# CliMA/OrthogonalSphericalShellGrids.jl

Hardware: AMD Instinct MI355X
Metric: grid-cells/s metric precompute + zipper halo-fill GB/s, 1/10°×75z (higher is better)
Workload: dtype f64

## Files before the change

orthogonalsphericalshellgrids.jl_amd/csrc/tpg_api.hip:

```cpp
#include "tpg_common.hpp"
#include <string.h>
#include <stdlib.h>
#include <atomic>
#include <mutex>

namespace tpg {

static thread_local char g_err[512] = "";

void set_error(const char* fmt, ...)
{
    va_list ap;
    va_start(ap, fmt);
    vsnprintf(g_err, sizeof(g_err), fmt, ap);
    va_end(ap);
}

#ifdef TPG_TEST_ABI
static std::atomic<const Config*> g_config{nullptr};
static std::mutex g_config_mutex;

static int env_int(const char* name, int dflt)
{
    const char* e = getenv(name);
    return (e && *e) ? atoi(e) : dflt;
}

static const Config* read_config()
{
    Config* c = new Config;
    c->cells_variant = env_int("TPG_CELLS_VARIANT", 2) == 0 ? 0 : 2;
    c->build_nt = env_int("TPG_BUILD_NT", 1) != 0;
    c->zipper_variant = env_int("TPG_ZIPPER_VARIANT", 3) == 0 ? 0 : 3;
    c->fill_fused = env_int("TPG_FILL_FUSED", -1);
    c->fill_merged = env_int("TPG_FILL_MERGED", -1);
    c->exchange_in_capture = env_int("TPG_EXCHANGE_IN_CAPTURE", 0) != 0;
    c->exchange_fail_stage = env_int("TPG_EXCHANGE_FAIL_STAGE", -1);
    const char* lib = getenv("TPG_RCCL_LIBRARY");
    c->rccl_library = (lib && *lib) ? strdup(lib) : nullptr;
    return c;
}

const Config& config()
{
    const Config* c = g_config.load(std::memory_order_acquire);
    if (!c) {
        std::lock_guard<std::mutex> lock(g_config_mutex);
        c = g_config.load(std::memory_order_acquire);
        if (!c) { c = read_config(); g_config.store(c, std::memory_order_release); }
    }
    return *c;
}
#else
const Config& config()
{
    static const Config k{ 2, true, 3, -1, -1, false, -1, nullptr };
    return k;
}
#endif

int check_geom(int Nx, int Ny, int Nz, int Hx, int Hy, int Hz, int ft)
{
    if (ft != TPG_F32 && ft != TPG_F64) { set_error("unknown element type ft=%d", ft); return TPG_ERR_INVALID_ARGUMENT; }
    if (Nx < 2 || Ny < 1 || Nz < 1 || Hx < 0 || Hy < 0 || Hz < 0) {
        set_error("invalid size (%d,%d,%d) / halo (%d,%d,%d)", Nx, Ny, Nz, Hx, Hy, Hz);
        return TPG_ERR_INVALID_ARGUMENT;
    }
    if (Nx % 2) {
        set_error("The number of cells in the longitude dimension should be even!");
        return TPG_ERR_ODD_NLAMBDA;
    }
    if (Hx > Nx || Hy > Ny) {
        set_error("halo (%d,%d) larger than size (%d,%d)", Hx, Hy, Nx, Ny);
        return TPG_ERR_UNSUPPORTED;
    }
    if ((long long)(Nx + 2 * Hx) * (Ny + 2 * Hy) >= (1ll << 31) || (long long)Nx * (Nz + 2 * Hz) * (Hy + 1) >= (1ll << 31)) {
        set_error("horizontal plane too large for 32-bit indexing");
        return TPG_ERR_UNSUPPORTED;
    }
    return TPG_OK;
}

}

extern "C" {

int tpg_version(void) { return TPG_VERSION; }

#ifdef TPG_TEST_ABI
int tpg_reload_config(void)
{
    std::lock_guard<std::mutex> lock(tpg::g_config_mutex);
    tpg::g_config.store(tpg::read_config(), std::memory_order_release);
    return TPG_OK;
}
#endif

const char* tpg_last_error(void) { return tpg::g_err; }

const char* tpg_status_string(int status)
{
    switch (status) {
    case TPG_OK: return "ok";
    case TPG_ERR_INVALID_ARGUMENT: return "invalid argument";
    case TPG_ERR_ODD_NLAMBDA: return "The number of cells in the longitude dimension should be even!";
    case TPG_ERR_BAD_PARTITION: return "latitude band outside the global grid (only y-partitioning is supported)";
    case TPG_ERR_WORKSPACE: return "workspace missing or too small";
    case TPG_ERR_UNSUPPORTED: return "unsupported size";
    case TPG_ERR_NOT_NORTH: return "Zipper boundary condition is valid on the north side only";
    case TPG_ERR_RCCL: return "RCCL error (librccl missing or ncclResult_t failure)";
    default: return status > 0 ? hipGetErrorString((hipError_t)status) : "unknown status";
    }
}

}
```

orthogonalsphericalshellgrids.jl_amd/csrc/tpg_grid.hip:

```cpp
#include "tpg_common.hpp"
#include "tpg_math.hpp"
#include "tpg_batch.hpp"

using namespace tpgm;

namespace {

constexpr double kC180Pi = 180.0 / kPi;
constexpr double kC360Pi = 360.0 / kPi;

struct GridK {
    int Nx, Ny, Hx, Hy;
    int shift;
    int jstart, jend;
    int jm_lo, jm_hi;
    int sx, rows;
    int ft;
    double fplp90;
    double R;
    const double* ti;
    const double* tj;
    const double* ts;
};

struct OutPtrs { void* p[TPG_NUM_ARRAYS]; };

struct TableArgs {
    int Nx, Ny, Hy, shift, ft;
    double south, npl, R;
    double* ti; double* tj; double* ts;
};

__device__ double lambda_face(int i, int N, int ft)
{
    long long num = 360ll * (i - 1) - 180ll * N;
    if (ft == TPG_F32) return (double)((float)num / (float)N);
    return (double)num / (double)N;
}
__device__ double lambda_center(int i, int N, int ft)
{
    long long num = 360ll * (2ll * i - 1) - 360ll * N;
    if (ft == TPG_F32) return (double)((float)num / (float)(2ll * N));
    return (double)num / (double)(2ll * N);
}
__device__ double phi_center(int j, int N, double south)
{
    if (N == 1) return south;
    if (south == __builtin_rint(south) && absD(south) < 1e6) {
        long long s = (long long)south;
        long long num = s * (N - 1) + (90 - s) * (long long)(j - 1);
        return (double)num / (double)(N - 1);
    }
    dd step = dd_div(two_sum(90.0, -south), dd{ (double)(N - 1), 0.0 });
    dd v = dd_add(dd{ south, 0.0 }, dd_mul_d(step, (double)(j - 1)));
    return v.hi + v.lo;
}

__global__ __launch_bounds__(64) void k_tables(TableArgs t)
{
    int tid = blockIdx.x * blockDim.x + threadIdx.x;
    const double a = tand((90.0 - t.npl) / 2);
    if (tid < t.Nx) {
        int is = tid + 1;
        int i0 = is - t.shift; if (i0 < 1) i0 += t.Nx;
        double lf = lambda_face(i0, t.Nx, t.ft), lc = lambda_center(i0, t.Nx, t.ft);
        double slf = sind(lf), clf = cosd(lf), slc = sind(lc), clc = cosd(lc);
        if (t.ft == TPG_F32) {
            slf = (double)(float)slf; clf = (double)(float)clf; slc = (double)(float)slc; clc = (double)(float)clc;
        }
        t.ti[0 * t.Nx + tid] = a * slf;
        t.ti[1 * t.Nx + tid] = a * clf;
        t.ti[2 * t.Nx + tid] = a * slc;
        t.ti[3 * t.Nx + tid] = a * clc;
        return;
    }
    tid -= t.Nx;
    if (tid < 2 * t.Ny) {
        int face = tid < t.Ny;
        int j = (face ? tid : tid - t.Ny) + 1;
        double pc = phi_center(j, t.Ny, t.south);
        double phi = pc;
        if (face) {
            double dphi = t.Ny > 1 ? phi_center(2, t.Ny, t.south) - phi_center(1, t.Ny, t.south) : 0.0;
            phi = pc - dphi / 2;
        }
        double psi = asinhD(tand((90.0 - phi) / 2) / a);
        double sh, ch;
        sinh_cosh(psi, sh, ch);
        int base = face ? 0 : 2;
        t.tj[(base + 0) * t.Ny + (j - 1)] = sh;
        t.tj[(base + 1) * t.Ny + (j - 1)] = ch;
        return;
    }
    tid -= 2 * t.Ny;
    if (tid <= t.Hy) {
        int j = 1 - t.Hy + tid;
        const double south = t.south, R = t.R;
        const double dlam = 360.0 / (double)t.Nx;
        const double dphiL = (90.0 - south) / (double)t.Ny;
        double pf, pfn, pc, pcm;
        if (south == __builtin_rint(south)) {
            long long s = (long long)south, Ny = t.Ny;
            pf  = (double)(s * Ny + (90 - s) * (long long)(j - 1)) / (double)Ny;
            pfn = (double)(s * Ny + (90 - s) * (long long)j) / (double)Ny;
            pc  = (double)(2 * s * Ny + (90 - s) * (long long)(2 * j - 1)) / (double)(2 * Ny);
            pcm = (double)(2 * s * Ny + (90 - s) * (long long)(2 * j - 3)) / (double)(2 * Ny);
        } else {
            pf  = south + (double)(j - 1) * dphiL;
            pfn = south + (double)j * dphiL;
            pc  = south + ((double)(2 * j - 1) * (90.0 - south)) / (double)(2 * t.Ny);
            pcm = south + ((double)(2 * j - 3) * (90.0 - south)) / (double)(2 * t.Ny);
        }
        int n = t.Hy + 1;
        t.ts[0 * n + tid] = R * (dlam * kDeg2Rad) * cosD(kPi * pc / 180);
        t.ts[1 * n + tid] = R * (dlam * kDeg2Rad) * cosD(kPi * pf / 180);
        t.ts[2 * n + tid] = R * R * (dlam * kDeg2Rad) * (sinD(kPi * pfn / 180) - sinD(kPi * pf / 180));
        t.ts[3 * n + tid] = R * R * (dlam * kDeg2Rad) * (sinD(kPi * pc / 180) - sinD(kPi * pcm / 180));
        t.ts[4 * n + tid] = R * (dphiL * kDeg2Rad);
    }
}

struct LP { double lam, phi; };

__device__ __forceinline__ LP analytic(const GridK& g, int xl, int yl, int is, int js)
{
    int i0 = is - g.shift; if (i0 < 1) i0 += g.Nx;
    const double* ti = g.ti + (xl == TPG_FACE ? 0 : 2) * g.Nx;
    const double* tj = g.tj + (yl == TPG_FACE ? 0 : 2) * g.Ny;
    double asl = ti[is - 1], acl = ti[g.Nx + is - 1];
    double sh = tj[js - 1], ch = tj[g.Ny + js - 1];
    double x = asl * ch;
    double y = acl * sh;
    bool pole = (x == 0.0) & (y == 0.0);
    double l = pole ? (i0 == 1 ? -90.0 : 90.0) : -kC180Pi * atanD(y / x);
    LP r;
    r.phi = 90.0 - kC360Pi * atanD(sqrt(y * y + x * x));
    l += (i0 <= g.Nx / 2) ? -90.0 : 90.0;
    l += g.fplp90;
    r.lam = fmod360(fmod360(l) + 360.0);
    return r;
}

__device__ __forceinline__ int fold_partner(int xl, int i, int Nx)
{
    int ip = (xl == TPG_FACE) ? Nx - i + 2 : Nx - i + 1;
    return ip > Nx ? ip - Nx : ip;
}

__device__ __forceinline__ LP coord(const GridK& g, int xl, int yl, int i, int j)
{
    if (j < 1) return LP{ 0.0, 0.0 };
    int iw = i < 1 ? i + g.Nx : (i > g.Nx ? i - g.Nx : i);
    int js = j;
    if (j > g.Ny) {
        int dj = j - g.Ny;
        js = (yl == TPG_FACE) ? g.Ny - dj + 1 : g.Ny - dj;
        iw = fold_partner(xl, iw, g.Nx);
        if (js < 1) return LP{ 0.0, 0.0 };
    } else if (j == g.Ny && yl == TPG_CENTER && iw > g.Nx / 2) {
        iw = fold_partner(xl, iw, g.Nx);
    }
    return analytic(g, xl, yl, iw, js);
}

__device__ __forceinline__ double haversine(LP a, LP b, double R)
{
    double dl = (b.lam - a.lam) * kDeg2Rad;
    double a1 = a.phi * kDeg2Rad;
    double a2 = b.phi * kDeg2Rad;
    double dp = a2 - a1;
    double s1 = sinD(dp / 2), s2 = sinD(dl / 2);
    double h = s1 * s1 + cosD(a1) * cosD(a2) * (s2 * s2);
    double r = sqrt(h);
    return 2 * (R * asinD(r != r ? r : (r < 1.0 ? r : 1.0)));
}

struct V3 { double x, y, z; };
__device__ __forceinline__ V3 cartesian(LP p)
{
    double cl = cosd(p.phi);
    return V3{ cosd(p.lam) * cl, sind(p.lam) * cl, sind(p.phi) };
}
__device__ __forceinline__ double dot3(V3 a, V3 b) { return a.x * b.x + a.y * b.y + a.z * b.z; }
__device__ __forceinline__ V3 cross3(V3 a, V3 b)
{
    return V3{ a.y * b.z - a.z * b.y, a.z * b.x - a.x * b.z, a.x * b.y - a.y * b.x };
}
__device__ __forceinline__ double tri_area(V3 a, V3 b, V3 c)
{
    double t = absD(dot3(a, cross3(b, c)));
    t /= 1 + dot3(a, b) + dot3(b, c) + dot3(a, c);
    return 2 * atanD(t);
}
__device__ __forceinline__ double quad_area(V3 a, V3 b, V3 c, V3 d)
{
    double A = tri_area(a, b, c);
    A += tri_area(a, b, d);
    A += tri_area(a, c, d);
    A += tri_area(b, c, d);
    return A / 2;
}

__device__ __forceinline__ double tri_tan_nr(V3 a, V3 b, V3 c)
{
    return div_nr(absD(dot3(a, cross3(b, c))), 1 + dot3(a, b) + dot3(b, c) + dot3(a, c));
}
__device__ __forceinline__ double tri_tan(V3 a, V3 b, V3 c)
{
    return absD(dot3(a, cross3(b, c))) / (1 + dot3(a, b) + dot3(b, c) + dot3(a, c));
}

template <typename T, bool NT = false>
__device__ __forceinline__ void put(const OutPtrs& o, int q, long long off, double v)
{
    T* p = static_cast<T*>(o.p[q]) + off;
    if (NT) __builtin_nontemporal_store((T)v, p); else *p = (T)v;
}

template <typename T, bool NT = false>
__device__ __forceinline__ void put32(const OutPtrs& o, int q, unsigned boff, double v)
{
    asm volatile("" : "+v"(boff));
    T* p = reinterpret_cast<T*>(static_cast<char*>(o.p[q]) + boff);
    if (NT) __builtin_nontemporal_store((T)v, p); else *p = (T)v;
}

template <typename T, bool NT>
__global__ __launch_bounds__(256) void k_cells(GridK g, OutPtrs o)
{
    const int nbx = (g.Nx + 255) / 256;
    int rb = blockIdx.x / nbx;
    int i = (blockIdx.x - rb * nbx) * 256 + threadIdx.x + 1;
    int j = g.jm_lo + rb;
    if (i > g.Nx) return;

    LP cc = coord(g, 0, 0, i, j), fc = coord(g, 1, 0, i, j), cf = coord(g, 0, 1, i, j), ff = coord(g, 1, 1, i, j);
    LP fc_e = coord(g, 1, 0, i + 1, j), fc_s = coord(g, 1, 0, i, j - 1);
    LP cc_w = coord(g, 0, 0, i - 1, j), cc_s = coord(g, 0, 0, i, j - 1), cc_sw = coord(g, 0, 0, i - 1, j - 1);
    LP ff_e = coord(g, 1, 1, i + 1, j), ff_n = coord(g, 1, 1, i, j + 1), ff_ne = coord(g, 1, 1, i + 1, j + 1);
    LP cf_w = coord(g, 0, 1, i - 1, j), cf_n = coord(g, 0, 1, i, j + 1);

    const double R = g.R;
    double dxcc = haversine(fc_e, fc, R);
    double dxfc = haversine(cc, cc_w, R);
    double dxcf = haversine(ff_e, ff, R);
    double dxff = haversine(cf, cf_w, R);
    double dycc = haversine(cf_n, cf, R);
    double dyfc = haversine(ff_n, ff, R);
    double dycf = haversine(cc, cc_s, R);
    double dyff = haversine(fc, fc_s, R);
    double azcc = quad_area(cartesian(ff), cartesian(ff_e), cartesian(ff_ne), cartesian(ff_n)) * (R * R);
    double azfc = dyfc * dxfc;
    double azcf = dycf * dxcf;
    double azff = quad_area(cartesian(cc_sw), cartesian(cc_s), cartesian(cc), cartesian(cc_w)) * (R * R);

    long long off = (long long)(i + g.Hx - 1) + (long long)g.sx * (j - g.jstart + g.Hy);
    put<T, NT>(o, TPG_LAMBDA_CC, off, cc.lam); put<T, NT>(o, TPG_LAMBDA_FC, off, fc.lam);
    put<T, NT>(o, TPG_LAMBDA_CF, off, cf.lam); put<T, NT>(o, TPG_LAMBDA_FF, off, ff.lam);
    put<T, NT>(o, TPG_PHI_CC, off, cc.phi); put<T, NT>(o, TPG_PHI_FC, off, fc.phi);
    put<T, NT>(o, TPG_PHI_CF, off, cf.phi); put<T, NT>(o, TPG_PHI_FF, off, ff.phi);
    put<T, NT>(o, TPG_DX_CC, off, dxcc); put<T, NT>(o, TPG_DX_FC, off, dxfc);
    put<T, NT>(o, TPG_DX_CF, off, dxcf); put<T, NT>(o, TPG_DX_FF, off, dxff);
    put<T, NT>(o, TPG_DY_CC, off, dycc); put<T, NT>(o, TPG_DY_CF, off, dycf);
    put<T, NT>(o, TPG_DY_FC, off, dyfc); put<T, NT>(o, TPG_DY_FF, off, dyff);
    put<T, NT>(o, TPG_AZ_CC, off, azcc); put<T, NT>(o, TPG_AZ_FC, off, azfc);
    put<T, NT>(o, TPG_AZ_CF, off, azcf); put<T, NT>(o, TPG_AZ_FF, off, azff);
}

struct Pt  { double lam, phi, a, ca; };
struct PtX { double lam, phi, a, ca, X, Y, Z; };
struct Nb  { double lam, a, ca; };
struct NbX { double lam, a, ca, X, Y, Z; };

__device__ __forceinline__ Pt make_pt(const GridK& g, int xl, int yl, int i, int j)
{
    LP p = coord(g, xl, yl, i, j);
    Pt r; r.lam = p.lam; r.phi = p.phi; r.a = p.phi * kDeg2Rad; r.ca = cosD(r.a);
    return r;
}
__device__ __forceinline__ PtX make_ptx(const GridK& g, int xl, int yl, int i, int j)
{
    LP p = coord(g, xl, yl, i, j);
    PtX r; r.lam = p.lam; r.phi = p.phi; r.a = p.phi * kDeg2Rad; r.ca = cosD(r.a);
    double sl, cl, sp, cp;
    sincosd(p.lam, sl, cl);
    sincosd(p.phi, sp, cp);
    r.X = cl * cp; r.Y = sl * cp; r.Z = sp;
    return r;
}
__device__ __forceinline__ Nb nb_of(const Pt& p) { return Nb{ p.lam, p.a, p.ca }; }
__device__ __forceinline__ Nb nb_of(const PtX& p) { return Nb{ p.lam, p.a, p.ca }; }
__device__ __forceinline__ NbX nbx_of(const PtX& p) { return NbX{ p.lam, p.a, p.ca, p.X, p.Y, p.Z }; }
__device__ __forceinline__ V3 v3_of(const PtX& p) { return V3{ p.X, p.Y, p.Z }; }
__device__ __forceinline__ V3 v3_of(const NbX& p) { return V3{ p.X, p.Y, p.Z }; }

template <int DIR> __device__ __forceinline__ double shf(double v)
{
    return DIR > 0 ? __shfl_down(v, 1, 64) : __shfl_up(v, 1, 64);
}
template <int DIR> __device__ __forceinline__ Nb shf_nb(const Pt& p)
{
    return Nb{ shf<DIR>(p.lam), shf<DIR>(p.a), shf<DIR>(p.ca) };
}
template <int DIR> __device__ __forceinline__ NbX shf_nbx(const PtX& p)
{
    return NbX{ shf<DIR>(p.lam), shf<DIR>(p.a), shf<DIR>(p.ca), shf<DIR>(p.X), shf<DIR>(p.Y), shf<DIR>(p.Z) };
}

__device__ __forceinline__ double hav(double xlam, double xa, double xca, double ylam, double ya, double yca, double R)
{
    double dl = (ylam - xlam) * kDeg2Rad;
    double dp = ya - xa;
    double s1 = sinD(dp / 2), s2 = sinD(dl / 2);
    double h = s1 * s1 + xca * yca * (s2 * s2);
    double r = sqrt(h);
    return 2 * (R * asinD(r != r ? r : (r < 1.0 ? r : 1.0)));
}
#define HAV(P, Q) hav((P).lam, (P).a, (P).ca, (Q).lam, (Q).a, (Q).ca, R)


struct Step4 {
    double lam[4], phi[4], a[4], ca[4];
    double X[2], Y[2], Z[2];
};

struct LaneConst { double aslF, aclF, aslC, aclC, hemi; };

struct RowTab { double shC, chC, shF, chF; };

typedef const double __attribute__((address_space(4))) kconst_double;
__device__ __forceinline__ RowTab load_rowtab(const GridK& g, int jc, int jf)
{
    kconst_double* tj = (kconst_double*)g.tj;
    jc = __builtin_amdgcn_readfirstlane(jc < 1 ? 1 : (jc > g.Ny ? g.Ny : jc));
    jf = __builtin_amdgcn_readfirstlane(jf < 1 ? 1 : (jf > g.Ny ? g.Ny : jf));
    return RowTab{ tj[2 * g.Ny + jc - 1], tj[3 * g.Ny + jc - 1], tj[0 * g.Ny + jf - 1], tj[1 * g.Ny + jf - 1] };
}

__device__ __forceinline__ void points_fast(const GridK& g, const LaneConst& lc, const RowTab& rt, Step4& s, const double* atab)
{
    const double shC = rt.shC, chC = rt.chC, shF = rt.shF, chF = rt.chF;
    double x[4] = { lc.aslF * chC, lc.aslC * chC, lc.aslF * chF, lc.aslC * chF };
    double y[4] = { lc.aclF * shC, lc.aclC * shC, lc.aclF * shF, lc.aclC * shF };
    double q[4], rr[4], at1[4], at2[4];
#pragma unroll
    for (int k = 0; k < 4; ++k) { q[k] = y[k] / x[k]; rr[k] = sqrt_nr<true>(y[k] * y[k] + x[k] * x[k]);    }
    tpgb::atan_tab_b<4>(q, at1, atab);
    tpgb::atan_tab_b<4, true>(rr, at2, atab);
#pragma unroll
    for (int k = 0; k < 4; ++k) {
        double l = -kC180Pi * at1[k];
        s.phi[k] = 90.0 - kC360Pi * at2[k];
        l += lc.hemi;
        l += g.fplp90;
        s.lam[k] = tpgb::fmod360_pos(tpgb::fmod360_small(l) + 360.0);
        s.a[k] = s.phi[k] * kDeg2Rad;
    }
    if (tpgb::cos_b<4>(s.a, s.ca)) {
#pragma unroll
        for (int k = 0; k < 4; ++k) s.ca[k] = cosD(s.a[k]);
    }
    double ang[4] = { s.lam[1], s.phi[1], s.lam[2], s.phi[2] }, sn[4], cs[4];
    tpgb::sincosd_b<4>(ang, sn, cs);
    s.X[0] = cs[0] * cs[1]; s.Y[0] = sn[0] * cs[1]; s.Z[0] = sn[1];
    s.X[1] = cs[2] * cs[3]; s.Y[1] = sn[2] * cs[3]; s.Z[1] = sn[3];
}

__device__ __forceinline__ void points_fast2(const GridK& g, const LaneConst& lc, const RowTab& rt, Step4& s, const double* atab)
{
    const double shC = rt.shC, chC = rt.chC, shF = rt.shF, chF = rt.chF;
    double x[4] = { lc.aslF * chC, lc.aslC * chC, lc.aslF * chF, lc.aslC * chF };
    double y[4] = { lc.aclF * shC, lc.aclC * shC, lc.aclF * shF, lc.aclC * shF };
    double q[4], rr[4], at1[4], at2[4];
    bool zerox = false;
#pragma unroll
    for (int k = 0; k < 4; ++k) { q[k] = div_nr(y[k], x[k]); zerox |= x[k] == 0.0; rr[k] = sqrt_nr<true>(y[k] * y[k] + x[k] * x[k]);    }
#pragma unroll
    for (int h = 0; h < 4; h += 2) {
        double qa[2] = { q[h], q[h + 1] }, ra[2] = { rr[h], rr[h + 1] }, o1[2], o2[2];
        tpgb::atan_tab_b<2, true>(qa, o1, atab);
        tpgb::atan_tab_b<2, true>(ra, o2, atab);
        at1[h] = o1[0]; at1[h + 1] = o1[1]; at2[h] = o2[0]; at2[h + 1] = o2[1];
    }
    if (zerox) {
#pragma unroll
        for (int k = 0; k < 4; ++k)
            if (x[k] == 0.0) {
                const double qq = y[k] / x[k];
                at1[k] = (qq != qq) ? qq : csign(kPio2Hi, qq);
            }
    }
#pragma unroll
    for (int k = 0; k < 4; ++k) {
        double l = -kC180Pi * at1[k];
        s.phi[k] = 90.0 - kC360Pi * at2[k];
        l += lc.hemi;
        l += g.fplp90;
        s.lam[k] = tpgb::fmod360_pos(tpgb::fmod360_small(l) + 360.0);
        s.a[k] = s.phi[k] * kDeg2Rad;
    }
    double sn[4], cs[4];
#pragma unroll
    for (int h = 0; h < 4; h += 2) {
        double aa[2] = { s.a[h], s.a[h + 1] }, cc2[2];
        if (tpgb::cos_lat_b<2>(aa, cc2)) { cc2[0] = cosD(aa[0]); cc2[1] = cosD(aa[1]); }
        s.ca[h] = cc2[0]; s.ca[h + 1] = cc2[1];
    }
    {
        double lon[2] = { s.lam[1], s.lam[2] }, lat[2] = { s.phi[1], s.phi[2] }, sl[2], cl[2], sp[2], cp[2];
        tpgb::sincosd_b<2>(lon, sl, cl);
        if (tpgb::sincosd_lat_b<2>(lat, sp, cp)) tpgb::sincosd_b<2>(lat, sp, cp);
        sn[0] = sl[0]; cs[0] = cl[0]; sn[1] = sp[0]; cs[1] = cp[0];
        sn[2] = sl[1]; cs[2] = cl[1]; sn[3] = sp[1]; cs[3] = cp[1];
    }
    s.X[0] = cs[0] * cs[1]; s.Y[0] = sn[0] * cs[1]; s.Z[0] = sn[1];
    s.X[1] = cs[2] * cs[3]; s.Y[1] = sn[2] * cs[3]; s.Z[1] = sn[3];
}

__device__ __noinline__ void points_general(const GridK& g, int i, int jc, int jf, Step4& s)
{
    Pt fc = make_pt(g, 1, 0, i, jc), cf = make_pt(g, 0, 1, i, jf);
    PtX cc = make_ptx(g, 0, 0, i, jc), ff = make_ptx(g, 1, 1, i, jf);
    s.lam[0] = fc.lam; s.phi[0] = fc.phi; s.a[0] = fc.a; s.ca[0] = fc.ca;
    s.lam[1] = cc.lam; s.phi[1] = cc.phi; s.a[1] = cc.a; s.ca[1] = cc.ca;
    s.lam[2] = ff.lam; s.phi[2] = ff.phi; s.a[2] = ff.a; s.ca[2] = ff.ca;
    s.lam[3] = cf.lam; s.phi[3] = cf.phi; s.a[3] = cf.a; s.ca[3] = cf.ca;
    s.X[0] = cc.X; s.Y[0] = cc.Y; s.Z[0] = cc.Z;
    s.X[1] = ff.X; s.Y[1] = ff.Y; s.Z[1] = ff.Z;
}

template <int R> struct TileLds { double v[18][R][64]; };
enum { L_FC = 0, L_CC = 3, L_FF = 9, L_CF = 15 };

template <int N>
__device__ __forceinline__ void hav_batch(const Nb (&X)[N], const Nb (&Y)[N], double Rad, double (&d)[N])
{
    double hp[N], hl[N], s1[N], s2[N], hh[N], rt[N], rm[N], as[N];
    bool zero = false;
#pragma unroll
    for (int e = 0; e < N; ++e) {
        double dp = Y[e].a - X[e].a;
        hp[e] = dp / 2; hl[e] = (Y[e].lam - X[e].lam) * (kDeg2Rad * 0.5);
    }
    if (tpgb::sin_small_b<N>(hp, s1)) {
#pragma unroll
        for (int e = 0; e < N; ++e) s1[e] = sinD(hp[e]);
    }
    if (tpgb::sin_small_b<N>(hl, s2)) {
#pragma unroll
        for (int e = 0; e < N; ++e) s2[e] = sinD(hl[e]);
    }
#pragma unroll
    for (int e = 0; e < N; ++e) {
        double h = s1[e] * s1[e] + X[e].ca * Y[e].ca * (s2[e] * s2[e]);
        hh[e] = h;
        zero |= h == 0.0;
        rt[e] = sqrt_nr<true>(h);
    }
    if (zero) {
#pragma unroll
        for (int e = 0; e < N; ++e) rt[e] = sqrt_nr(hh[e]);
    }
#pragma unroll
    for (int e = 0; e < N; ++e) {
        rm[e] = __builtin_fmin(rt[e], 1.0);
    }
    if (tpgb::asin_small_b<N>(rm, as)) {
#pragma unroll
        for (int e = 0; e < N; ++e) as[e] = asinD(!(rt[e] >= 1.0) ? rt[e] : 1.0);
    }
#pragma unroll
    for (int e = 0; e < N; ++e) d[e] = (2 * Rad) * as[e];
}

template <typename T, bool NT, int R>
__global__ __launch_bounds__(64 * R, 4) void k_cells_tile(GridK g, OutPtrs o, int tiles_x)
{
    __shared__ __attribute__((aligned(16))) double atabs[R][TPG_ATAN_TABLE_DOUBLES];
    __shared__ TileLds<R> lds;
    const int lane = threadIdx.x & 63;
    const int p = __builtin_amdgcn_readfirstlane(threadIdx.x >> 6);
    double* atab = atabs[p];
    tpgb::atan_table_init(atab, lane);
    __builtin_amdgcn_fence(__ATOMIC_RELEASE, "wavefront");
    __builtin_amdgcn_wave_barrier();
    __builtin_amdgcn_fence(__ATOMIC_ACQUIRE, "wavefront");
    const int ty = (int)gridDim.y - 1 - (int)blockIdx.y;
    const int tx = blockIdx.x;
    const int s0 = g.jm_lo - 1 + ty * (R - 1);
    const int s = s0 + p;
    int i = tx * 62 + lane;
    const bool col_emit = lane >= 1 && lane <= 62 && i <= g.Nx;
    if (i > g.Nx + 1) i = g.Nx + 1;
    const double Rad = g.R;
    const bool active_row = s <= g.jm_hi;
    const unsigned col = (unsigned)(i + g.Hx - 1);
    auto rowoff = [&](int j) -> unsigned { return (col + (unsigned)g.sx * (unsigned)(j - g.jstart + g.Hy)) * (unsigned)sizeof(T); };

    Step4 q;
    if (active_row) {
        const bool fast = s >= 1 && s < g.Ny && absD(g.fplp90) <= 360.0;
        if (fast) {
            LaneConst lc;
            const int iw = i < 1 ? i + g.Nx : (i > g.Nx ? i - g.Nx : i);
            int i0 = iw - g.shift; if (i0 < 1) i0 += g.Nx;
            lc.aslF = g.ti[0 * g.Nx + iw - 1]; lc.aclF = g.ti[1 * g.Nx + iw - 1];
            lc.aslC = g.ti[2 * g.Nx + iw - 1]; lc.aclC = g.ti[3 * g.Nx + iw - 1];
            lc.hemi = (i0 <= g.Nx / 2) ? -90.0 : 90.0;
            points_fast2(g, lc, load_rowtab(g, s, s + 1), q, atab);
        } else {
            Step4 tmp; GridK gc = g; points_general(gc, i, s, s + 1, tmp); q = tmp;
        }
        if (col_emit) {
            if (p >= 1 && s >= g.jm_lo) {
                unsigned off = rowoff(s);
                put32<T, NT>(o, TPG_LAMBDA_FC, off, q.lam[0]); put32<T, NT>(o, TPG_PHI_FC, off, q.phi[0]);
                put32<T, NT>(o, TPG_LAMBDA_CC, off, q.lam[1]); put32<T, NT>(o, TPG_PHI_CC, off, q.phi[1]);
            }
            if ((p >= 1 || ty == 0) && s + 1 >= g.jm_lo && s + 1 <= g.jm_hi) {
                unsigned off1 = rowoff(s + 1);
                put32<T, NT>(o, TPG_LAMBDA_FF, off1, q.lam[2]); put32<T, NT>(o, TPG_PHI_FF, off1, q.phi[2]);
                put32<T, NT>(o, TPG_LAMBDA_CF, off1, q.lam[3]); put32<T, NT>(o, TPG_PHI_CF, off1, q.phi[3]);
            }
        }
        double (*L)[R][64] = lds.v;
        L[L_FC + 0][p][lane] = q.lam[0]; L[L_FC + 1][p][lane] = q.a[0]; L[L_FC + 2][p][lane] = q.ca[0];
        L[L_CC + 0][p][lane] = q.lam[1]; L[L_CC + 1][p][lane] = q.a[1]; L[L_CC + 2][p][lane] = q.ca[1];
        L[L_CC + 3][p][lane] = q.X[0];   L[L_CC + 4][p][lane] = q.Y[0]; L[L_CC + 5][p][lane] = q.Z[0];
        L[L_FF + 0][p][lane] = q.lam[2]; L[L_FF + 1][p][lane] = q.a[2]; L[L_FF + 2][p][lane] = q.ca[2];
        L[L_FF + 3][p][lane] = q.X[1];   L[L_FF + 4][p][lane] = q.Y[1]; L[L_FF + 5][p][lane] = q.Z[1];
        L[L_CF + 0][p][lane] = q.lam[3]; L[L_CF + 1][p][lane] = q.a[3]; L[L_CF + 2][p][lane] = q.ca[3];
    }
    __syncthreads();
    if (p == 0) {
        if (!col_emit) return;
        double (*L)[R][64] = lds.v;
#pragma unroll 1
        for (int r = 1; r < R; r += 2) {
            const int sa = s0 + r, sb = sa + 1;
            if (sa > g.jm_hi) break;
            const bool two = (r + 1 < R) && sb <= g.jm_hi;
            const int rb = two ? r + 1 : r;
            Nb X[2] = { Nb{ L[L_FC + 0][r][lane], L[L_FC + 1][r][lane], L[L_FC + 2][r][lane] },
                        Nb{ L[L_FC + 0][rb][lane], L[L_FC + 1][rb][lane], L[L_FC + 2][rb][lane] } };
            Nb Y[2] = { Nb{ L[L_FC + 0][r - 1][lane], L[L_FC + 1][r - 1][lane], L[L_FC + 2][r - 1][lane] },
                        Nb{ L[L_FC + 0][rb - 1][lane], L[L_FC + 1][rb - 1][lane], L[L_FC + 2][rb - 1][lane] } };
            double dd2[2];
            hav_batch<2>(X, Y, Rad, dd2);
            if (sa >= g.jm_lo) put32<T, NT>(o, TPG_DY_FF, rowoff(sa), dd2[0]);
            if (two && sb >= g.jm_lo) put32<T, NT>(o, TPG_DY_FF, rowoff(sb), dd2[1]);
        }
        return;
    }
    if (!active_row || s < g.jm_lo || !col_emit) return;

    double (*L)[R][64] = lds.v;
    const int pm = p - 1, le = lane + 1, lw = lane - 1;
    const unsigned off = rowoff(s);

#pragma unroll
    for (int k = 0; k < 2; ++k) {
        V3 a, b, c, dd;
        if (k == 0) {
            a = V3{ L[L_FF + 3][pm][lane], L[L_FF + 4][pm][lane], L[L_FF + 5][pm][lane] };
            b = V3{ L[L_FF + 3][pm][le], L[L_FF + 4][pm][le], L[L_FF + 5][pm][le] };
            c = V3{ L[L_FF + 3][p][le], L[L_FF + 4][p][le], L[L_FF + 5][p][le] };
            dd = V3{ q.X[1], q.Y[1], q.Z[1] };
        } else {
            a = V3{ L[L_CC + 3][pm][lw], L[L_CC + 4][pm][lw], L[L_CC + 5][pm][lw] };
            b = V3{ L[L_CC + 3][pm][lane], L[L_CC + 4][pm][lane], L[L_CC + 5][pm][lane] };
            c = V3{ q.X[0], q.Y[0], q.Z[0] };
            dd = V3{ L[L_CC + 3][p][lw], L[L_CC + 4][p][lw], L[L_CC + 5][p][lw] };
        }
        double tt[4], at[4];
        tt[0] = tri_tan_nr(a, b, c); tt[1] = tri_tan_nr(a, b, dd);
        tt[2] = tri_tan_nr(a, c, dd); tt[3] = tri_tan_nr(b, c, dd);
        if (__any(tpgb::atan_small_b<4>(tt, at))) {
            tt[0] = tri_tan(a, b, c); tt[1] = tri_tan(a, b, dd); tt[2] = tri_tan(a, c, dd); tt[3] = tri_tan(b, c, dd);
            tpgb::atan_b<4>(tt, at);
        }
        double A = at[0];
        A += at[1];
        A += at[2];
        A += at[3];
        put32<T, NT>(o, k == 0 ? TPG_AZ_CC : TPG_AZ_FF, off, A * (Rad * Rad));
    }

    auto ld = [&](int f, int pp, int ll) -> Nb { return Nb{ L[f + 0][pp][ll], L[f + 1][pp][ll], L[f + 2][pp][ll] }; };
    const Nb own[4] = { Nb{ q.lam[0], q.a[0], q.ca[0] }, Nb{ q.lam[1], q.a[1], q.ca[1] },
                        Nb{ q.lam[2], q.a[2], q.ca[2] }, Nb{ q.lam[3], q.a[3], q.ca[3] } };
    double d[8];
#pragma unroll
    for (int hb = 0; hb < 6; hb += 2) {
        Nb X[2], Y[2];
        if (hb == 0)      { X[0] = ld(L_FC, p, le); Y[0] = own[0];            X[1] = own[1];            Y[1] = ld(L_CC, p, lw); }
        else if (hb == 2) { X[0] = ld(L_FF, pm, le); Y[0] = ld(L_FF, pm, lane); X[1] = ld(L_CF, pm, lane); Y[1] = ld(L_CF, pm, lw); }
        else              { X[0] = own[3];           Y[0] = ld(L_CF, pm, lane); X[1] = own[2];            Y[1] = ld(L_FF, pm, lane); }
        double dd2[2];
        hav_batch<2>(X, Y, Rad, dd2);
        d[hb] = dd2[0]; d[hb + 1] = dd2[1];
    }
    {
        Nb X[1] = { own[1] }, Y[1] = { ld(L_CC, pm, lane) };
        double dd1[1];
        hav_batch<1>(X, Y, Rad, dd1);
        d[6] = dd1[0];
    }
    put32<T, NT>(o, TPG_DX_CC, off, d[0]); put32<T, NT>(o, TPG_DX_FC, off, d[1]);
    put32<T, NT>(o, TPG_DX_CF, off, d[2]); put32<T, NT>(o, TPG_DX_FF, off, d[3]);
    put32<T, NT>(o, TPG_DY_CC, off, d[4]); put32<T, NT>(o, TPG_DY_FC, off, d[5]);
    put32<T, NT>(o, TPG_DY_CF, off, d[6]);
    put32<T, NT>(o, TPG_AZ_FC, off, d[5] * d[1]);
    put32<T, NT>(o, TPG_AZ_CF, off, d[6] * d[2]);
}

__device__ __forceinline__ void array_loc(int q, int& xl, int& yl)
{
    int r = q & 3;
    bool dy = (q >= TPG_DY_CC && q <= TPG_DY_FF);
    int xr = dy ? (r >> 1) : (r & 1);
    int yr = dy ? (r & 1) : (r >> 1);
    xl = xr; yl = yr;
}

struct HaloRegions {
    int nA;
    int nB;
    int nC;
    int nD;
    int nsouth;
    int merged_south;
};

template <typename T>
__global__ __launch_bounds__(256) void k_halos(GridK g, OutPtrs o, HaloRegions h)
{
    int t = blockIdx.x * blockDim.x + threadIdx.x;
    int q = blockIdx.y;
    int xl, yl;
    array_loc(q, xl, yl);
    const bool is_coord = q < TPG_DX_CC;
    T* A = static_cast<T*>(o.p[q]);
    const long long sx = g.sx;
    auto at = [&](int i, int j) -> long long { return (long long)(i + g.Hx - 1) + sx * (j - g.jstart + g.Hy); };

    int i, j;
    if (t < h.nA) {
        int r = t / (2 * g.Hx), c = t - r * 2 * g.Hx;
        j = g.jm_lo + r;
        i = c < g.Hx ? 1 - g.Hx + c : g.Nx + 1 + (c - g.Hx);
        if (h.merged_south && !is_coord && j <= 1) return;
    } else if ((t -= h.nA) < h.nB) {
        int r = t / g.sx, c = t - r * g.sx;
        j = g.Ny + 1 + r; i = 1 - g.Hx + c;
    } else if ((t -= h.nB) < h.nC) {
        int r = t / g.sx, c = t - r * g.sx;
        j = 1 - h.nsouth + r; i = 1 - g.Hx + c;
        if (is_coord) { if (j < 1) A[at(i, j)] = (T)0; return; }
        if (!h.merged_south) return;
        const int n = g.Hy + 1, rt = j - (1 - g.Hy);
        const int col = (q >= TPG_DY_CC && q <= TPG_DY_FF) ? 4 : ((q >= TPG_AZ_CC ? 2 : 0) + (yl == TPG_FACE ? 1 : 0));
        A[at(i, j)] = (T)g.ts[col * n + rt];
        return;
    } else if ((t -= h.nC) < h.nD) {
        if (is_coord || yl != TPG_CENTER) return;
        i = g.Nx / 2 + 1 + t; j = g.Ny;
    } else {
        return;
    }

    int iw = i < 1 ? i + g.Nx : (i > g.Nx ? i - g.Nx : i);
    int js = j;
    if (j > g.Ny) {
        int dj = j - g.Ny;
        js = (yl == TPG_FACE) ? g.Ny - dj + 1 : g.Ny - dj;
        iw = fold_partner(xl, iw, g.Nx);
        if (js < 1) { A[at(i, j)] = (T)0; return; }
    } else if (j == g.Ny && yl == TPG_CENTER && iw > g.Nx / 2) {
        iw = fold_partner(xl, iw, g.Nx);
    }
    A[at(i, j)] = A[at(iw, js)];
}

template <typename T>
__global__ __launch_bounds__(256) void k_south(GridK g, OutPtrs o)
{
    int c = blockIdx.x * blockDim.x + threadIdx.x;
    int r = blockIdx.y;
    int lr = (1 - g.Hy + r) - (g.jstart - g.Hy);
    if (c >= g.sx || lr < 0 || lr >= g.rows) return;
    int n = g.Hy + 1;
    double dxc = g.ts[0 * n + r], dxf = g.ts[1 * n + r], azc = g.ts[2 * n + r], azf = g.ts[3 * n + r], dy = g.ts[4 * n + r];
    long long off = (long long)c + (long long)g.sx * lr;
    put<T>(o, TPG_DX_FF, off, dxf); put<T>(o, TPG_DX_FC, off, dxc); put<T>(o, TPG_DX_CF, off, dxf); put<T>(o, TPG_DX_CC, off, dxc);
    put<T>(o, TPG_DY_FF, off, dy);  put<T>(o, TPG_DY_FC, off, dy);  put<T>(o, TPG_DY_CF, off, dy);  put<T>(o, TPG_DY_CC, off, dy);
    put<T>(o, TPG_AZ_FF, off, azf); put<T>(o, TPG_AZ_FC, off, azc); put<T>(o, TPG_AZ_CF, off, azf); put<T>(o, TPG_AZ_CC, off, azc);
}

size_t table_doubles(const tpg_params* p) { return 4 * (size_t)p->Nx + 4 * (size_t)p->Ny + 5 * (size_t)(p->Hy + 1); }

int check_params(const tpg_params* p)
{
    if (!p) { tpg::set_error("null params"); return TPG_ERR_INVALID_ARGUMENT; }
    int rc = tpg::check_geom(p->Nx, p->Ny, p->Nz, p->Hx, p->Hy, p->Hz, p->ft);
    if (rc) return rc;
    if (p->jstart < 1 || p->jend > p->Ny || p->jend < p->jstart) {
        tpg::set_error("latitude band %d:%d outside 1:%d", p->jstart, p->jend, p->Ny);
        return TPG_ERR_BAD_PARTITION;
    }
    if (p->reserved & ~TPG_BUILD_TABLES_VALID) {
        tpg::set_error("tpg_params.reserved: unknown flag bits 0x%x", p->reserved & ~TPG_BUILD_TABLES_VALID);
        return TPG_ERR_INVALID_ARGUMENT;
    }
    if (!(p->radius > 0) || !(p->north_poles_latitude < 90) || !(p->southernmost_latitude < 90)) {
        tpg::set_error("invalid radius / latitudes");
        return TPG_ERR_INVALID_ARGUMENT;
    }
    return TPG_OK;
}

template <typename T>
int launch_build(const GridK& g, const OutPtrs& o, const HaloRegions& h, hipStream_t s)
{
    dim3 grid1(((g.Nx + 255) / 256) * (g.jm_hi - g.jm_lo + 1));
    const tpg::Config& cfg = tpg::config();
    const bool nt = cfg.build_nt;
    constexpr int R = 8;
    const int nrows = g.jm_hi - g.jm_lo + 1;
    const int tiles_y = (nrows + (R - 1) - 1) / (R - 1);
    const bool offsets32 = (unsigned long long)g.sx * (unsigned long long)(g.jend - g.jstart + 1 + 2 * g.Hy) * sizeof(T) < (1ull << 32);
    const bool south_in_band = g.jstart - g.Hy <= 1;
    const bool tile = cfg.cells_variant != 0 && tiles_y <= 65535 && offsets32;
    if (tile) {
        const int tiles_x = (g.Nx + 61) / 62;
        dim3 gridt((unsigned)tiles_x, (unsigned)tiles_y);
        if (nt) hipLaunchKernelGGL((k_cells_tile<T, true, R>), gridt, dim3(64 * R), 0, s, g, o, tiles_x);
        else    hipLaunchKernelGGL((k_cells_tile<T, false, R>), gridt, dim3(64 * R), 0, s, g, o, tiles_x);
    }
    else if (nt) hipLaunchKernelGGL((k_cells<T, true>), grid1, dim3(256), 0, s, g, o);
    else         hipLaunchKernelGGL((k_cells<T, false>), grid1, dim3(256), 0, s, g, o);
    int rc = tpg::launch_status("k_cells");
    if (rc) return rc;
    HaloRegions hm = h;
    hm.merged_south = (south_in_band && g.Ny > 2 * g.Hy + 2) ? 1 : 0;
    if (hm.merged_south) hm.nC = (h.nsouth + 1) * g.sx;
    int nh = hm.nA + hm.nB + hm.nC + hm.nD;
    if (nh > 0) {
        hipLaunchKernelGGL(k_halos<T>, dim3((nh + 255) / 256, TPG_NUM_ARRAYS), dim3(256), 0, s, g, o, hm);
        if ((rc = tpg::launch_status("k_halos"))) return rc;
    }
    if (south_in_band && !hm.merged_south) {
        hipLaunchKernelGGL(k_south<T>, dim3((g.sx + 255) / 256, g.Hy + 1), dim3(256), 0, s, g, o);
        if ((rc = tpg::launch_status("k_south"))) return rc;
    }
    return TPG_OK;
}

}

extern "C" {

size_t tpg_build_grid_workspace_bytes(const tpg_params* p)
{
    if (!p || p->Nx < 1 || p->Ny < 1 || p->Hy < 0) return 0;
    return (table_doubles(p) * sizeof(double) + 255) & ~(size_t)255;
}

int tpg_build_grid(const tpg_params* p, void* const out[TPG_NUM_ARRAYS], void* workspace,
                   size_t workspace_bytes, void* stream)
{
    int rc = check_params(p);
    if (rc) return rc;
    if (!out) { tpg::set_error("null output table"); return TPG_ERR_INVALID_ARGUMENT; }
    OutPtrs o;
    for (int q = 0; q < TPG_NUM_ARRAYS; ++q) {
        if (!out[q]) { tpg::set_error("null output array %d", q); return TPG_ERR_INVALID_ARGUMENT; }
        o.p[q] = out[q];
    }
    if (!workspace || workspace_bytes < table_doubles(p) * sizeof(double) || ((uintptr_t)workspace & 7)) {
        tpg::set_error("workspace: need %zu bytes, 8-byte aligned", table_doubles(p) * sizeof(double));
        return TPG_ERR_WORKSPACE;
    }
    hipStream_t s = tpg::as_stream(stream);
    double* w = static_cast<double*>(workspace);

    TableArgs t;
    t.Nx = p->Nx; t.Ny = p->Ny; t.Hy = p->Hy; t.shift = p->Nx / 4; t.ft = p->ft;
    t.south = p->southernmost_latitude; t.npl = p->north_poles_latitude; t.R = p->radius;
    t.ti = w; t.tj = w + 4 * (size_t)p->Nx; t.ts = t.tj + 4 * (size_t)p->Ny;
    if (!(p->reserved & TPG_BUILD_TABLES_VALID)) {
        int nt = p->Nx + 2 * p->Ny + p->Hy + 1;
        hipLaunchKernelGGL(k_tables, dim3((nt + 63) / 64), dim3(64), 0, s, t);
        if ((rc = tpg::launch_status("k_tables"))) return rc;
    }

    GridK g;
    g.Nx = p->Nx; g.Ny = p->Ny; g.Hx = p->Hx; g.Hy = p->Hy; g.shift = p->Nx / 4;
    g.jstart = p->jstart; g.jend = p->jend;
    g.jm_lo = p->jstart - p->Hy < 1 ? 1 : p->jstart - p->Hy;
    g.jm_hi = p->jend + p->Hy > p->Ny ? p->Ny : p->jend + p->Hy;
    g.sx = p->Nx + 2 * p->Hx; g.rows = p->jend - p->jstart + 1 + 2 * p->Hy;
    g.ft = p->ft; g.fplp90 = p->first_pole_longitude + 90.0; g.R = p->radius;
    g.ti = t.ti; g.tj = t.tj; g.ts = t.ts;

    HaloRegions h;
    h.nA = (g.jm_hi - g.jm_lo + 1) * 2 * g.Hx;
    h.nB = (p->jend + p->Hy > p->Ny) ? (p->jend + p->Hy - p->Ny) * g.sx : 0;
    h.nsouth = (1 - (p->jstart - p->Hy)) > 0 ? (1 - (p->jstart - p->Hy)) : 0;
    h.nC = h.nsouth * g.sx;
    h.nD = (p->jend + p->Hy >= p->Ny) ? p->Nx / 2 : 0;

    if (p->ft == TPG_F64) return launch_build<double>(g, o, h, s);
    return launch_build<float>(g, o, h, s);
}

}
```

Before: 11.93 billion.

## Pair mirror-symmetric columns in one wavefront to share transcendental work via lane permutes

Adds a paired tile mode, now the default, that maps the lower and upper 32 lanes of each wavefront to mirror-image columns across the tripolar fold. Each lane computes atan, cos and sincos for only one of the two symmetric point sets and takes the partner's results through ds_bpermute, roughly halving the transcendental math per cell. Each tile now covers 30 column pairs instead of 62 columns, so the grid layout and column-emit logic change. The costs are extra permute traffic, a special-case path for zero x that must stay correct, and reliance on the exact symmetry of the fold.

```diff
diff --git a/orthogonalsphericalshellgrids.jl_amd/csrc/tpg_api.hip b/orthogonalsphericalshellgrids.jl_amd/csrc/tpg_api.hip
--- a/orthogonalsphericalshellgrids.jl_amd/csrc/tpg_api.hip
+++ b/orthogonalsphericalshellgrids.jl_amd/csrc/tpg_api.hip
@@ -29,7 +29,8 @@
 static const Config* read_config()
 {
     Config* c = new Config;
-    c->cells_variant = env_int("TPG_CELLS_VARIANT", 2) == 0 ? 0 : 2;
+    const int cv = env_int("TPG_CELLS_VARIANT", 2);
+    c->cells_variant = (cv == 0 || cv == 1) ? cv : 2;
     c->build_nt = env_int("TPG_BUILD_NT", 1) != 0;
     c->zipper_variant = env_int("TPG_ZIPPER_VARIANT", 3) == 0 ? 0 : 3;
     c->fill_fused = env_int("TPG_FILL_FUSED", -1);
diff --git a/orthogonalsphericalshellgrids.jl_amd/csrc/tpg_grid.hip b/orthogonalsphericalshellgrids.jl_amd/csrc/tpg_grid.hip
--- a/orthogonalsphericalshellgrids.jl_amd/csrc/tpg_grid.hip
+++ b/orthogonalsphericalshellgrids.jl_amd/csrc/tpg_grid.hip
@@ -417,6 +417,69 @@
     s.X[1] = cs[2] * cs[3]; s.Y[1] = sn[2] * cs[3]; s.Z[1] = sn[3];
 }
 
+__device__ __forceinline__ double lane_pull(int addr, double v)
+{
+    const int lo = __builtin_amdgcn_ds_bpermute(addr, __double2loint(v));
+    const int hi = __builtin_amdgcn_ds_bpermute(addr, __double2hiint(v));
+    return __hiloint2double(hi, lo);
+}
+
+__device__ __forceinline__ void points_pair(const GridK& g, const LaneConst& lc, const RowTab& rt, Step4& s, const double* atab,
+                                            const bool up, const int addrF, const int addrC)
+{
+    const double shC = rt.shC, chC = rt.chC, shF = rt.shF, chF = rt.chF;
+    const bool zerox = (lc.aslF == 0.0) | (lc.aslC == 0.0);
+    const double aslS = up ? lc.aslF : lc.aslC, aclS = up ? lc.aclF : lc.aclC;
+    const double xs[2] = { aslS * chC, aslS * chF }, ys[2] = { aclS * shC, aclS * shF };
+    double qa[2], ra[2], o1[2], o2[2], ph[2], aa[2], cc2[2];
+#pragma unroll
+    for (int c = 0; c < 2; ++c) { qa[c] = div_nr(ys[c], xs[c]); ra[c] = sqrt_nr<true>(ys[c] * ys[c] + xs[c] * xs[c]); }
+    tpgb::atan_tab_b<2, true>(ra, o2, atab);
+    tpgb::atan_tab_b<2, true>(qa, o1, atab);
+    double at1[4];
+#pragma unroll
+    for (int k = 0; k < 4; ++k) at1[k] = lane_pull((k & 1) ? addrC : addrF, o1[k >> 1]);
+#pragma unroll
+    for (int c = 0; c < 2; ++c) { ph[c] = 90.0 - kC360Pi * o2[c]; aa[c] = ph[c] * kDeg2Rad; }
+    if (tpgb::cos_lat_b<2>(aa, cc2)) { cc2[0] = cosD(aa[0]); cc2[1] = cosD(aa[1]); }
+    double lat[1] = { up ? ph[1] : ph[0] }, sp[1], cp[1];
+    if (tpgb::sincosd_lat_b<1>(lat, sp, cp)) tpgb::sincosd_b<1>(lat, sp, cp);
+#pragma unroll
+    for (int k = 0; k < 4; ++k) {
+        const int addr = (k & 1) ? addrC : addrF, c = k >> 1;
+        s.phi[k] = lane_pull(addr, ph[c]);
+        s.ca[k] = lane_pull(addr, cc2[c]);
+    }
+    const double spCC = lane_pull(addrC, sp[0]), cpCC = lane_pull(addrC, cp[0]);
+    const double spFF = lane_pull(addrF, sp[0]), cpFF = lane_pull(addrF, cp[0]);
+    if (zerox) {
+        const double x[4] = { lc.aslF * chC, lc.aslC * chC, lc.aslF * chF, lc.aslC * chF };
+        const double y[4] = { lc.aclF * shC, lc.aclC * shC, lc.aclF * shF, lc.aclC * shF };
+#pragma unroll
+        for (int k = 0; k < 4; ++k)
+            if (x[k] == 0.0) {
+                const double qq = y[k] / x[k];
+                const double v = (qq != qq) ? qq : csign(kPio2Hi, qq);
+                at1[k] = (((k & 1) != 0) == up) ? -v : v;
+            }
+    }
+    const double cF = up ? -kC180Pi : kC180Pi, cC = -cF;
+#pragma unroll
+    for (int k = 0; k < 4; ++k) {
+        double l = ((k & 1) ? cC : cF) * at1[k];
+        l += lc.hemi;
+        l += g.fplp90;
+        s.lam[k] = tpgb::fmod360_pos(tpgb::fmod360_small(l) + 360.0);
+    }
+    double lon[2] = { s.lam[1], s.lam[2] }, sl[2], cl[2];
+    tpgb::sincosd_b<2>(lon, sl, cl);
+    __builtin_amdgcn_sched_barrier(0);
+#pragma unroll
+    for (int k = 0; k < 4; ++k) s.a[k] = s.phi[k] * kDeg2Rad;
+    s.X[0] = cl[0] * cpCC; s.Y[0] = sl[0] * cpCC; s.Z[0] = spCC;
+    s.X[1] = cl[1] * cpFF; s.Y[1] = sl[1] * cpFF; s.Z[1] = spFF;
+}
+
 __device__ __noinline__ void points_general(const GridK& g, int i, int jc, int jf, Step4& s)
 {
     Pt fc = make_pt(g, 1, 0, i, jc), cf = make_pt(g, 0, 1, i, jf);
@@ -473,7 +536,7 @@
     for (int e = 0; e < N; ++e) d[e] = (2 * Rad) * as[e];
 }
 
-template <typename T, bool NT, int R>
+template <typename T, bool NT, int R, bool PAIR>
 __global__ __launch_bounds__(64 * R, 4) void k_cells_tile(GridK g, OutPtrs o, int tiles_x)
 {
     __shared__ __attribute__((aligned(16))) double atabs[R][TPG_ATAN_TABLE_DOUBLES];
@@ -489,9 +552,20 @@
     const int tx = blockIdx.x;
     const int s0 = g.jm_lo - 1 + ty * (R - 1);
     const int s = s0 + p;
-    int i = tx * 62 + lane;
-    const bool col_emit = lane >= 1 && lane <= 62 && i <= g.Nx;
-    if (i > g.Nx + 1) i = g.Nx + 1;
+    int i;
+    bool col_emit;
+    const bool up = lane >= 32;
+    if (PAIR) {
+        const int hl = lane & 31, half = g.Nx >> 1, a = tx * 30 + 1;
+        int i0 = (up ? g.Nx - a - 29 : a - 1) + hl;
+        col_emit = hl >= 1 && hl <= 30 && (up ? i0 > half : i0 <= half);
+        if (i0 < 1 || i0 > g.Nx) i0 = up ? 1 : g.Nx;
+        i = i0 + g.shift; if (i > g.Nx) i -= g.Nx;
+    } else {
+        i = tx * 62 + lane;
+        col_emit = lane >= 1 && lane <= 62 && i <= g.Nx;
+        if (i > g.Nx + 1) i = g.Nx + 1;
+    }
     const double Rad = g.R;
     const bool active_row = s <= g.jm_hi;
     const unsigned col = (unsigned)(i + g.Hx - 1);
@@ -507,7 +581,8 @@
             lc.aslF = g.ti[0 * g.Nx + iw - 1]; lc.aclF = g.ti[1 * g.Nx + iw - 1];
             lc.aslC = g.ti[2 * g.Nx + iw - 1]; lc.aclC = g.ti[3 * g.Nx + iw - 1];
             lc.hemi = (i0 <= g.Nx / 2) ? -90.0 : 90.0;
-            points_fast2(g, lc, load_rowtab(g, s, s + 1), q, atab);
+            if (PAIR) points_pair(g, lc, load_rowtab(g, s, s + 1), q, atab, up, (up ? lane : (64 - lane) & 63) << 2, (up ? 63 - lane : lane) << 2);
+            else points_fast2(g, lc, load_rowtab(g, s, s + 1), q, atab);
         } else {
             Step4 tmp; GridK gc = g; points_general(gc, i, s, s + 1, tmp); q = tmp;
         }
@@ -731,11 +806,17 @@
     const bool offsets32 = (unsigned long long)g.sx * (unsigned long long)(g.jend - g.jstart + 1 + 2 * g.Hy) * sizeof(T) < (1ull << 32);
     const bool south_in_band = g.jstart - g.Hy <= 1;
     const bool tile = cfg.cells_variant != 0 && tiles_y <= 65535 && offsets32;
-    if (tile) {
+    if (tile && cfg.cells_variant == 2) {
+        const int tiles_x = (g.Nx / 2 + 29) / 30;
+        dim3 gridt((unsigned)tiles_x, (unsigned)tiles_y);
+        if (nt) hipLaunchKernelGGL((k_cells_tile<T, true, R, true>), gridt, dim3(64 * R), 0, s, g, o, tiles_x);
+        else    hipLaunchKernelGGL((k_cells_tile<T, false, R, true>), gridt, dim3(64 * R), 0, s, g, o, tiles_x);
+    }
+    else if (tile) {
         const int tiles_x = (g.Nx + 61) / 62;
         dim3 gridt((unsigned)tiles_x, (unsigned)tiles_y);
-        if (nt) hipLaunchKernelGGL((k_cells_tile<T, true, R>), gridt, dim3(64 * R), 0, s, g, o, tiles_x);
-        else    hipLaunchKernelGGL((k_cells_tile<T, false, R>), gridt, dim3(64 * R), 0, s, g, o, tiles_x);
+        if (nt) hipLaunchKernelGGL((k_cells_tile<T, true, R, false>), gridt, dim3(64 * R), 0, s, g, o, tiles_x);
+        else    hipLaunchKernelGGL((k_cells_tile<T, false, R, false>), gridt, dim3(64 * R), 0, s, g, o, tiles_x);
     }
     else if (nt) hipLaunchKernelGGL((k_cells<T, true>), grid1, dim3(256), 0, s, g, o);
     else         hipLaunchKernelGGL((k_cells<T, false>), grid1, dim3(256), 0, s, g, o);
```

After: 10.53 billion. 11.7% lower.

## Exploit tripolar mirror symmetry to share atan/cos work between paired columns

Applied to the files above, without the earlier changes.

Reorganises the tiled cell kernel so each wavefront covers mirrored column pairs: the lower half-wave handles columns east of the shift and the upper half handles the mirror columns to the west. Each lane computes only two of the four point atans, cosines and lat sincos, exchanges them through LDS, and rebuilds the mirrored atan values by flipping sign bits. The goal is to roughly halve the transcendental work per cell. The cost is extra LDS traffic, extra wave barriers, new column-wrapping index math, and a reliance on exact symmetry of the input tables. Results would be wrong if Nx is odd or if the tables are not symmetric.

```diff
diff --git a/orthogonalsphericalshellgrids.jl_amd/csrc/tpg_grid.hip b/orthogonalsphericalshellgrids.jl_amd/csrc/tpg_grid.hip
--- a/orthogonalsphericalshellgrids.jl_amd/csrc/tpg_grid.hip
+++ b/orthogonalsphericalshellgrids.jl_amd/csrc/tpg_grid.hip
@@ -366,55 +366,80 @@
     s.X[1] = cs[2] * cs[3]; s.Y[1] = sn[2] * cs[3]; s.Z[1] = sn[3];
 }
 
-__device__ __forceinline__ void points_fast2(const GridK& g, const LaneConst& lc, const RowTab& rt, Step4& s, const double* atab)
-{
-    const double shC = rt.shC, chC = rt.chC, shF = rt.shF, chF = rt.chF;
-    double x[4] = { lc.aslF * chC, lc.aslC * chC, lc.aslF * chF, lc.aslC * chF };
-    double y[4] = { lc.aclF * shC, lc.aclC * shC, lc.aclF * shF, lc.aclC * shF };
-    double q[4], rr[4], at1[4], at2[4];
-    bool zerox = false;
-#pragma unroll
-    for (int k = 0; k < 4; ++k) { q[k] = div_nr(y[k], x[k]); zerox |= x[k] == 0.0; rr[k] = sqrt_nr<true>(y[k] * y[k] + x[k] * x[k]);    }
-#pragma unroll
-    for (int h = 0; h < 4; h += 2) {
-        double qa[2] = { q[h], q[h + 1] }, ra[2] = { rr[h], rr[h + 1] }, o1[2], o2[2];
-        tpgb::atan_tab_b<2, true>(qa, o1, atab);
-        tpgb::atan_tab_b<2, true>(ra, o2, atab);
-        at1[h] = o1[0]; at1[h + 1] = o1[1]; at2[h] = o2[0]; at2[h + 1] = o2[1];
-    }
-    if (zerox) {
-#pragma unroll
-        for (int k = 0; k < 4; ++k)
-            if (x[k] == 0.0) {
-                const double qq = y[k] / x[k];
-                at1[k] = (qq != qq) ? qq : csign(kPio2Hi, qq);
-            }
-    }
+template <int R>
+__device__ __forceinline__ void points_pair(const GridK& g, const LaneConst& lc, const RowTab& rt, Step4& s, const double* atab,
+                                            double (*L)[R][64], int p, int lane)
+{
+    const bool face = lane >= 32;
+    const double aslO = face ? lc.aslF : lc.aslC, aclO = face ? lc.aclF : lc.aclC;
+    {
+        const double x[2] = { aslO * rt.chC, aslO * rt.chF };
+        const double y[2] = { aclO * rt.shC, aclO * rt.shF };
+        double q[2], rr[2], at1[2], at2[2], phi[2], a[2], ca[2];
+        bool zerox = false;
+#pragma unroll
+        for (int m = 0; m < 2; ++m) { q[m] = div_nr(y[m], x[m]); zerox |= x[m] == 0.0; rr[m] = sqrt_nr<true>(y[m] * y[m] + x[m] * x[m]);    }
+        tpgb::atan_tab_b<2, true>(q, at1, atab);
+        tpgb::atan_tab_b<2, true>(rr, at2, atab);
+        if (zerox) {
+#pragma unroll
+            for (int m = 0; m < 2; ++m)
+                if (x[m] == 0.0) {
+                    const double qq = y[m] / x[m];
+                    at1[m] = (qq != qq) ? qq : csign(kPio2Hi, qq);
+                }
+        }
+#pragma unroll
+        for (int m = 0; m < 2; ++m) { phi[m] = 90.0 - kC360Pi * at2[m]; a[m] = phi[m] * kDeg2Rad; }
+        if (tpgb::cos_lat_b<2>(a, ca)) { ca[0] = cosD(a[0]); ca[1] = cosD(a[1]); }
+        double lat[1] = { face ? phi[1] : phi[0] }, sp[1], cp[1];
+        if (tpgb::sincosd_lat_b<1>(lat, sp, cp)) tpgb::sincosd_b<1>(lat, sp, cp);
+        const int k0 = face ? 0 : 1;
+        L[3 * k0 + 0][p][lane] = at1[0]; L[3 * k0 + 1][p][lane] = phi[0]; L[3 * k0 + 2][p][lane] = ca[0];
+        L[3 * k0 + 6][p][lane] = at1[1]; L[3 * k0 + 7][p][lane] = phi[1]; L[3 * k0 + 8][p][lane] = ca[1];
+        L[14 - 2 * k0][p][lane] = sp[0]; L[15 - 2 * k0][p][lane] = cp[0];
+    }
+    __builtin_amdgcn_fence(__ATOMIC_RELEASE, "wavefront");
+    __builtin_amdgcn_wave_barrier();
+    __builtin_amdgcn_fence(__ATOMIC_ACQUIRE, "wavefront");
+    const int srcF = face ? lane : (lane == 0 ? 63 : 64 - lane), srcC = face ? 63 - lane : lane;
+    const int sgF = __double2hiint(lc.aslF) ^ __double2hiint(lc.aclF), sgC = __double2hiint(lc.aslC) ^ __double2hiint(lc.aclC);
+    const int sgJc = __double2hiint(rt.shC), sgJf = __double2hiint(rt.shF);
+    const int sg[4] = { sgF ^ sgJc, sgC ^ sgJc, sgF ^ sgJf, sgC ^ sgJf };
+    double at1[4], sp[2], cp[2];
+#pragma unroll
+    for (int k = 0; k < 4; ++k) {
+        const int src = (k == 0 || k == 2) ? srcF : srcC;
+        const double t = L[3 * k + 0][p][src];
+        at1[k] = __hiloint2double((__double2hiint(t) & 0x7fffffff) | (sg[k] & (int)0x80000000), __double2loint(t));
+        s.phi[k] = L[3 * k + 1][p][src];
+        s.ca[k] = L[3 * k + 2][p][src];
+    }
+    sp[0] = L[12][p][srcC]; cp[0] = L[13][p][srcC];
+    sp[1] = L[14][p][srcF]; cp[1] = L[15][p][srcF];
+    __builtin_amdgcn_fence(__ATOMIC_RELEASE, "wavefront");
+    __builtin_amdgcn_wave_barrier();
+    __builtin_amdgcn_fence(__ATOMIC_ACQUIRE, "wavefront");
 #pragma unroll
     for (int k = 0; k < 4; ++k) {
         double l = -kC180Pi * at1[k];
-        s.phi[k] = 90.0 - kC360Pi * at2[k];
         l += lc.hemi;
         l += g.fplp90;
         s.lam[k] = tpgb::fmod360_pos(tpgb::fmod360_small(l) + 360.0);
         s.a[k] = s.phi[k] * kDeg2Rad;
     }
-    double sn[4], cs[4];
-#pragma unroll
-    for (int h = 0; h < 4; h += 2) {
-        double aa[2] = { s.a[h], s.a[h + 1] }, cc2[2];
-        if (tpgb::cos_lat_b<2>(aa, cc2)) { cc2[0] = cosD(aa[0]); cc2[1] = cosD(aa[1]); }
-        s.ca[h] = cc2[0]; s.ca[h + 1] = cc2[1];
-    }
-    {
-        double lon[2] = { s.lam[1], s.lam[2] }, lat[2] = { s.phi[1], s.phi[2] }, sl[2], cl[2], sp[2], cp[2];
-        tpgb::sincosd_b<2>(lon, sl, cl);
-        if (tpgb::sincosd_lat_b<2>(lat, sp, cp)) tpgb::sincosd_b<2>(lat, sp, cp);
-        sn[0] = sl[0]; cs[0] = cl[0]; sn[1] = sp[0]; cs[1] = cp[0];
-        sn[2] = sl[1]; cs[2] = cl[1]; sn[3] = sp[1]; cs[3] = cp[1];
-    }
-    s.X[0] = cs[0] * cs[1]; s.Y[0] = sn[0] * cs[1]; s.Z[0] = sn[1];
-    s.X[1] = cs[2] * cs[3]; s.Y[1] = sn[2] * cs[3]; s.Z[1] = sn[3];
+    double lon[2] = { s.lam[1], s.lam[2] }, sl[2], cl[2];
+    tpgb::sincosd_b<2>(lon, sl, cl);
+    s.X[0] = cl[0] * cp[0]; s.Y[0] = sl[0] * cp[0]; s.Z[0] = sp[0];
+    s.X[1] = cl[1] * cp[1]; s.Y[1] = sl[1] * cp[1]; s.Z[1] = sp[1];
+}
+
+__device__ __forceinline__ int wrap_col(int v, int Nx)
+{
+    if (v < 1) v += Nx;
+    if (v > Nx) v -= Nx;
+    if (v < 1 || v > Nx) { v = (v - 1) % Nx; v = (v < 0 ? v + Nx : v) + 1; }
+    return v;
 }
 
 __device__ __noinline__ void points_general(const GridK& g, int i, int jc, int jf, Step4& s)
@@ -489,9 +514,9 @@
     const int tx = blockIdx.x;
     const int s0 = g.jm_lo - 1 + ty * (R - 1);
     const int s = s0 + p;
-    int i = tx * 62 + lane;
-    const bool col_emit = lane >= 1 && lane <= 62 && i <= g.Nx;
-    if (i > g.Nx + 1) i = g.Nx + 1;
+    const int hl = lane & 31;
+    const int i = wrap_col(lane >= 32 ? g.shift - 30 * tx - 30 + hl : g.shift + 30 * tx + hl, g.Nx);
+    const bool col_emit = hl >= 1 && hl <= 30 && 30 * tx + (lane >= 32 ? 30 - hl : hl - 1) < g.Nx / 2;
     const double Rad = g.R;
     const bool active_row = s <= g.jm_hi;
     const unsigned col = (unsigned)(i + g.Hx - 1);
@@ -502,12 +527,11 @@
         const bool fast = s >= 1 && s < g.Ny && absD(g.fplp90) <= 360.0;
         if (fast) {
             LaneConst lc;
-            const int iw = i < 1 ? i + g.Nx : (i > g.Nx ? i - g.Nx : i);
-            int i0 = iw - g.shift; if (i0 < 1) i0 += g.Nx;
-            lc.aslF = g.ti[0 * g.Nx + iw - 1]; lc.aclF = g.ti[1 * g.Nx + iw - 1];
-            lc.aslC = g.ti[2 * g.Nx + iw - 1]; lc.aclC = g.ti[3 * g.Nx + iw - 1];
+            int i0 = i - g.shift; if (i0 < 1) i0 += g.Nx;
+            lc.aslF = g.ti[0 * g.Nx + i - 1]; lc.aclF = g.ti[1 * g.Nx + i - 1];
+            lc.aslC = g.ti[2 * g.Nx + i - 1]; lc.aclC = g.ti[3 * g.Nx + i - 1];
             lc.hemi = (i0 <= g.Nx / 2) ? -90.0 : 90.0;
-            points_fast2(g, lc, load_rowtab(g, s, s + 1), q, atab);
+            points_pair<R>(g, lc, load_rowtab(g, s, s + 1), q, atab, lds.v, p, lane);
         } else {
             Step4 tmp; GridK gc = g; points_general(gc, i, s, s + 1, tmp); q = tmp;
         }
@@ -732,7 +756,7 @@
     const bool south_in_band = g.jstart - g.Hy <= 1;
     const bool tile = cfg.cells_variant != 0 && tiles_y <= 65535 && offsets32;
     if (tile) {
-        const int tiles_x = (g.Nx + 61) / 62;
+        const int tiles_x = (g.Nx / 2 + 29) / 30;
         dim3 gridt((unsigned)tiles_x, (unsigned)tiles_y);
         if (nt) hipLaunchKernelGGL((k_cells_tile<T, true, R>), gridt, dim3(64 * R), 0, s, g, o, tiles_x);
         else    hipLaunchKernelGGL((k_cells_tile<T, false, R>), gridt, dim3(64 * R), 0, s, g, o, tiles_x);
```

Result: faster. 11.98 billion before, 12.61 billion after (median of 6 runs) (+5.3%).
